# Unalome81/IEEE-802.11-OFDM-QPSK-Simulator

Measured on NVIDIA B200. Metric: OFDM symbols/s, TX+AWGN+RX chain (BER/EVM sweep), higher is better.
Workload: dtype f32+f64

## Files before the change

ieee-802.11-ofdm-qpsk-simulator_b200/binding.py:

```python
import ctypes as C
import os

import numpy as np

HERE = os.path.dirname(os.path.abspath(__file__))
LIB_PATH = os.path.join(HERE, "libofdm_b200.so")

MODE_EXACT, MODE_FAST = 0, 1
NFFT, CP, SYM_LEN, LTS_LEN, DATA_PER_SYM, BITS_PER_SYM, WORDS_PER_SYM = 64, 16, 80, 160, 48, 96, 3


def frame_len(n_sym):
    return LTS_LEN + SYM_LEN * n_sym


class Counters(C.Structure):
    _fields_ = [("bit_errors", C.c_uint64), ("bits", C.c_uint64), ("frames_in_error", C.c_uint64),
                ("rail_errors", C.c_uint64), ("frames", C.c_uint64),
                ("sum_err2", C.c_double), ("sum_ref2", C.c_double), ("sum_evm_lin", C.c_double)]

    def as_dict(self):
        return {k: getattr(self, k) for k, _ in self._fields_}

    def __iadd__(self, o):
# ... 31 lines not shown
    pass


_VP, _I, _L, _F, _U32, _U64, _SZ = C.c_void_p, C.c_int, C.c_long, C.c_float, C.c_uint32, C.c_uint64, C.c_size_t

SIGNATURES = {
    "ofdm_version": (_I, []),
    "ofdm_strerror": (C.c_char_p, [_I]),
    "ofdm_ctx_create": (_I, [C.POINTER(_VP), _I]),
    "ofdm_ctx_destroy": (_I, [_VP]),
    "ofdm_last_error": (C.c_char_p, [_VP]),
    "ofdm_ctx_set_stream": (_I, [_VP, _VP]),
    "ofdm_ctx_stream": (_VP, [_VP]),
    "ofdm_ctx_sync": (_I, [_VP]),
    "ofdm_ctx_set_option": (_I, [_VP, C.c_char_p, _I]),
    "ofdm_ctx_replayed_frames": (_I, [_VP, C.POINTER(_U64), _I]),
    "ofdm_ctx_sm_count": (_I, [_VP]),
    "ofdm_ctx_launch_count": (_U64, [_VP]),
    "ofdm_dev_alloc": (_I, [_VP, C.POINTER(_VP), _SZ]),
    "ofdm_dev_free": (_I, [_VP, _VP]),
    "ofdm_host_alloc": (_I, [_VP, C.POINTER(_VP), _SZ]),
    "ofdm_host_free": (_I, [_VP, _VP]),
    "ofdm_memcpy_h2d": (_I, [_VP, _VP, _VP, _SZ]),
    "ofdm_memcpy_d2h": (_I, [_VP, _VP, _VP, _SZ]),
    "ofdm_memset_dev": (_I, [_VP, _VP, _I, _SZ]),
    "ofdm_pack_bits": (_I, [_VP, _VP, _VP, _L]),
    "ofdm_unpack_bits": (_I, [_VP, _VP, _VP, _L]),
    "ofdm_qpsk_modulate": (_I, [_VP, _VP, _VP, _L]),
    "ofdm_map_subcarriers": (_I, [_VP, _VP, _VP, _L]),
    "ofdm_ifft64": (_I, [_VP, _VP, _VP, _L, _I]),
    "ofdm_fft64": (_I, [_VP, _VP, _VP, _L, _I]),
    "ofdm_add_cp": (_I, [_VP, _VP, _VP, _L]),
    "ofdm_lts": (_I, [_VP, _VP, _VP]),
    "ofdm_tx_frames": (_I, [_VP, _VP, _VP, _VP, _L, _I, _I]),
    "ofdm_frame_power": (_I, [_VP, _VP, _VP, _L, _I, _I]),
    "ofdm_awgn_inject": (_I, [_VP, _VP, _VP, _VP, _F, _VP, _L, _I, _I]),
    "ofdm_awgn_philox": (_I, [_VP, _VP, _VP, _F, _U32, _U32, _U64, _VP, _L, _I, _I]),
    "ofdm_awgn_philox_ex": (_I, [_VP, _I, _I, _VP, _VP, _F, _U32, _U32, _U64, _VP, _L, _I, _I]),
    "ofdm_rx_frames": (_I, [_VP, _VP, _VP, _L, _I, _I, _VP, C.POINTER(RxDump)]),
    "ofdm_awgn_rx_inject": (_I, [_VP, _VP, _VP, _VP, _VP, _F, _L, _I, _I, _VP, C.POINTER(RxDump)]),
    "ofdm_awgn_rx_philox": (_I, [_VP, _VP, _VP, _VP, _F, _U32, _U32, _U64, _L, _I, _I, _VP, C.POINTER(RxDump)]),
    "ofdm_awgn_rx_inject_sweep": (_I, [_VP, _VP, _VP, _VP, _VP, _VP, _I, _L, _I, _I, _VP]),
    "ofdm_strip_cp": (_I, [_VP, _VP, _VP, _L, _I, _I, _I]),
    "ofdm_channel_estimate": (_I, [_VP, _VP, _VP, _L, _I, _I, _I]),
    "ofdm_equalize": (_I, [_VP, _VP, _VP, _VP, _L, _I, _I]),
    "ofdm_demap": (_I, [_VP, _VP, _VP, _L]),
    "ofdm_agc_slicer": (_I, [_VP, _VP, _VP, _L]),
    "ofdm_qpsk_demodulate": (_I, [_VP, _VP, _VP, _L]),
    "ofdm_sweep_inject_host": (_I, [_VP, _VP, _VP, _L, _I, _VP, _I, _I, C.POINTER(Counters)]),
    "ofdm_sweep_inject_dev": (_I, [_VP, _VP, _VP, _L, _I, _VP, _I, _I, C.POINTER(Counters)]),
    "ofdm_random_bits": (_I, [_VP, _U32, _U64, _L, _I, _VP]),
    "ofdm_mc_sweep_philox_dev": (_I, [_VP, _U32, _U64, _L, _I, _VP, _I, _I, _VP]),
    "ofdm_mc_sweep_points_dev": (_I, [_VP, _U32, _U64, _L, _I, _I, _VP, _VP, _I, _I, _VP]),
    "ofdm_mc_sweep_until": (_I, [_VP, _U32, _U64, _I, _I, _VP, _I, _I, _U64, _U64, _L, C.POINTER(Counters), C.POINTER(_I)]),
    "ofdm_mc_sweep_channel_dev": (_I, [_VP, C.POINTER(Channel), _U32, _U64, _L, _I, _VP, _VP, _I, _I, _VP]),
    "ofdm_mc_sweep_channel_until": (_I, [_VP, C.POINTER(Channel), _U32, _U64, _I, _VP, _I, _I, _U64, _U64, _L, C.POINTER(Counters),
                                         C.POINTER(_I)]),
    "ofdm_mc_sweep_philox": (_I, [_VP, _U32, _U64, _L, _I, _VP, _I, _I, C.POINTER(Counters)]),
    "ofdm_multipath_taps": (_I, [_VP, _VP, _VP, _I, _VP, _L, _I]),
    "ofdm_multipath_philox": (_I, [_VP, _VP, _U32, _U64, _I, _VP, _VP, _L, _I]),
    "ofdm_mc_sweep_multipath_dev": (_I, [_VP, _U32, _U64, _L, _I, _I, _VP, _I, _I, _VP]),
    "ofdm_rrc_tx": (_I, [_VP, _VP, _VP, _L, _I]),
    "ofdm_rrc_rx": (_I, [_VP, _VP, _VP, _L, _I, _I, _I]),
    "ofdm_awgn_inject_len": (_I, [_VP, _VP, _VP, _VP, _F, _VP, _L, _I, _I]),
    "ofdm_packet_detect": (_I, [_VP, _VP, _VP, _L, _I]),
    "ofdm_packet_select": (_I, [_VP, _VP, _VP, _L, _I]),
# ... 447 lines not shown
```

ieee-802.11-ofdm-qpsk-simulator_b200/csrc/ofdm_b200.cu:

```cuda
#include <cmath>
#include <cstdio>
#include <cstdlib>
#include <cstring>
#include <mutex>
#include <new>
#include <set>
#include <type_traits>
#include <utility>

#include "ofdm_chain.cuh"
#include "ofdm_stream.cuh"
#include "ofdm_mc_quad.cuh"
#include "ofdm_sweep.cuh"

using namespace ofdm;

struct ofdm_ctx {
    int device = 0;
    int sm_count = 0;
    cudaStream_t stream = nullptr;
    bool owns_stream = false;
    cudaStream_t copy_stream = nullptr;
    cudaEvent_t copy_done[2] = {nullptr, nullptr}, call_start = nullptr;
    uint64_t launches = 0;
// ... 85 lines not shown
int stream_grid(ofdm_ctx *ctx, long rows, int rows_per_block, int per_sm)
{
    const long need = (rows + rows_per_block - 1) / rows_per_block, full = (long)per_sm * ctx->sm_count;
    const long g = need < full ? need : full;
    return (int)(g < 1 ? 1 : g);
}

int ensure_scratch(ofdm_ctx *ctx, int slot, size_t bytes, void **out)
{
    if (ctx->scratch_bytes[slot] < bytes) {
        if (ctx->scratch[slot]) { cudaFree(ctx->scratch[slot]); ctx->scratch[slot] = nullptr; ctx->scratch_bytes[slot] = 0; }
        cudaError_t e = cudaMalloc(&ctx->scratch[slot], bytes);
        if (e != cudaSuccess) return fail(ctx, OFDM_ERR_NOMEM, "cudaMalloc(scratch)", e);
        ctx->scratch_bytes[slot] = bytes;
    }
    *out = ctx->scratch[slot];
    return OFDM_OK;
}

float snr_linear(float snr_db)
{
    return (float)pow(10.0, (double)(snr_db / 10));
}

__global__ void k_power_prefix(const float2 *__restrict__ x, int n, float *__restrict__ out)
{
    float p = 0.f;
    for (int i = 0; i < n; ++i) {
        const double h = hypot_glibc((double)x[i].x, (double)x[i].y);
        p = __double2float_rn(__dadd_rn((double)p, __dmul_rn(h, h)));
    }
    *out = p;
}

struct DeviceTables {
    bool ready = false;
    float lts_freq[128], lts_time[320], sts_time[320], lts_power_prefix;
};
std::mutex g_tables_mutex;
DeviceTables g_tables[64];

int upload_tables(ofdm_ctx *ctx, const float *lts_time , float power_prefix)
{
    Tables t;
    memset(&t, 0, sizeof t);
    for (int k = 0; k < 32; ++k) t.tw64[k] = make_double2(kTw64[k][0], kTw64[k][1]);
    for (int k = 0; k < 64; ++k) {
        double a = 2.0 * 3.14159265358979323846 * k / 64.0;
        t.tw64f[k] = make_float2((float)cos(a), (float)(-sin(a)));
    }
    signed char by_c[64];
    for (int c = 0; c < 64; ++c) by_c[c] = -1;
    const int lo[6] = {6, 12, 26, 33, 40, 54}, hi[6] = {10, 24, 31, 38, 52, 58};
    int d = 0;
    for (int r = 0; r < 6; ++r) for (int c = lo[r]; c <= hi[r]; ++c) by_c[c] = (signed char)d++;
    by_c[11] = -2; by_c[25] = -2; by_c[39] = -2; by_c[53] = -3;
    for (int p = 0; p < 64; ++p) {
        int c = (p + 32) & 63;
        t.bin_data[p] = by_c[c];
        t.bin_lts[p] = (c >= 6 && c <= 58) ? kLk[c - 6] : 0;
        if (by_c[c] >= 0) t.data_bin[by_c[c]] = (int8_t)p;
    }
    if (lts_time) {
        memcpy(t.lts_time, lts_time, sizeof t.lts_time);
        double sum = 0.0;
        for (int i = 0; i < 160; ++i) sum += (double)lts_time[2 * i] * lts_time[2 * i] + (double)lts_time[2 * i + 1] * lts_time[2 * i + 1];
// ... 185 lines not shown
    std::lock_guard<std::mutex> lock(g_tables_mutex);
    DeviceTables &dt = g_tables[device & 63];
    int st = OFDM_OK;
    float *d_buf = nullptr;
    if (dt.ready) {
        memcpy(ctx->lts_freq, dt.lts_freq, sizeof dt.lts_freq);
        memcpy(ctx->lts_time, dt.lts_time, sizeof dt.lts_time);
        memcpy(ctx->sts_time, dt.sts_time, sizeof dt.sts_time);
        ctx->lts_power_prefix = dt.lts_power_prefix;
    } else {
    st = upload_tables(ctx, nullptr, 0.f);
    if (st == OFDM_OK && cudaMalloc(&d_buf, (2 * 128 + 320 + 4) * sizeof(float)) != cudaSuccess) st = OFDM_ERR_NOMEM;
    if (st == OFDM_OK) {
        memset(ctx->lts_freq, 0, sizeof ctx->lts_freq);
        for (int i = 0; i < 53; ++i) ctx->lts_freq[2 * (6 + i)] = (float)kLk[i];
        float t64[128];
        if (cudaMemcpyAsync(d_buf, ctx->lts_freq, sizeof ctx->lts_freq, cudaMemcpyHostToDevice, ctx->stream) != cudaSuccess) st = OFDM_ERR_CUDA;
        if (st == OFDM_OK) st = launch_fft<true, true>(ctx, d_buf, d_buf + 128, 1);
        if (st == OFDM_OK && cudaMemcpyAsync(t64, d_buf + 128, sizeof t64, cudaMemcpyDeviceToHost, ctx->stream) != cudaSuccess) st = OFDM_ERR_CUDA;
        if (st == OFDM_OK && cudaStreamSynchronize(ctx->stream) != cudaSuccess) st = OFDM_ERR_CUDA;
        if (st == OFDM_OK) {
            memcpy(ctx->lts_time, t64 + 64, 32 * 2 * sizeof(float));
            memcpy(ctx->lts_time + 64, t64, 64 * 2 * sizeof(float));
            memcpy(ctx->lts_time + 64 + 128, t64, 64 * 2 * sizeof(float));
            float *d_lts = d_buf + 256, *d_pref = d_buf + 256 + 320;
            if (cudaMemcpyAsync(d_lts, ctx->lts_time, sizeof ctx->lts_time, cudaMemcpyHostToDevice, ctx->stream) != cudaSuccess) st = OFDM_ERR_CUDA;
            if (st == OFDM_OK) {
                k_power_prefix<<<1, 1, 0, ctx->stream>>>(reinterpret_cast<const float2 *>(d_lts), 160, d_pref);
                st = check_launch(ctx, "k_power_prefix");
            }
            if (st == OFDM_OK && cudaMemcpyAsync(&ctx->lts_power_prefix, d_pref, sizeof(float), cudaMemcpyDeviceToHost, ctx->stream) != cudaSuccess) st = OFDM_ERR_CUDA;
            if (st == OFDM_OK && cudaStreamSynchronize(ctx->stream) != cudaSuccess) st = OFDM_ERR_CUDA;
            if (st == OFDM_OK) st = upload_tables(ctx, ctx->lts_time, ctx->lts_power_prefix);
        }
    }
    if (st == OFDM_OK) {
        static const signed char Sk[53] = {0,0,1,0,0,0,-1,0,0,0, 1,0,0,0,-1,0,0,0,-1,0,0,0, 1,0,0,0,0,0,0,0,-1,0,0,0, -1,0,0,0,1,0,0,0,1,0,0,0, 1,0,0,0,1,0,0};
        const float scale = (float)sqrt(13.0 / 6.0);
        float grid[128], t64[128];
        memset(grid, 0, sizeof grid);
        for (int i = 0; i < 53; ++i) { grid[2 * (6 + i)] = (float)Sk[i] * scale; grid[2 * (6 + i) + 1] = (float)Sk[i] * scale; }
        if (cudaMemcpyAsync(d_buf, grid, sizeof grid, cudaMemcpyHostToDevice, ctx->stream) != cudaSuccess) st = OFDM_ERR_CUDA;
        if (st == OFDM_OK) st = launch_fft<true, true>(ctx, d_buf, d_buf + 128, 1);
        if (st == OFDM_OK && cudaMemcpyAsync(t64, d_buf + 128, sizeof t64, cudaMemcpyDeviceToHost, ctx->stream) != cudaSuccess) st = OFDM_ERR_CUDA;
        if (st == OFDM_OK && cudaStreamSynchronize(ctx->stream) != cudaSuccess) st = OFDM_ERR_CUDA;
        if (st == OFDM_OK) for (int r = 0; r < 10; ++r) memcpy(ctx->sts_time + 32 * r, t64, 16 * 2 * sizeof(float));
    }
    if (st == OFDM_OK) {
        memcpy(dt.lts_freq, ctx->lts_freq, sizeof dt.lts_freq);
        memcpy(dt.lts_time, ctx->lts_time, sizeof dt.lts_time);
        memcpy(dt.sts_time, ctx->sts_time, sizeof dt.sts_time);
        dt.lts_power_prefix = ctx->lts_power_prefix;
        dt.ready = true;
    }
    }
    if (st == OFDM_OK) {
        if (cudaMalloc(&ctx->replayed_dev, sizeof(unsigned long long)) != cudaSuccess) st = OFDM_ERR_NOMEM;
        else if (cudaMemset(ctx->replayed_dev, 0, sizeof(unsigned long long)) != cudaSuccess) st = OFDM_ERR_CUDA;
    }
    if (st == OFDM_OK) {
        if (cudaMalloc(&ctx->sts_dev, sizeof ctx->sts_time) != cudaSuccess) st = OFDM_ERR_NOMEM;
        else if (cudaMemcpy(ctx->sts_dev, ctx->sts_time, sizeof ctx->sts_time, cudaMemcpyHostToDevice) != cudaSuccess) st = OFDM_ERR_CUDA;
    }
    if (d_buf) cudaFree(d_buf);
    if (st != OFDM_OK) { ofdm_ctx_destroy(ctx); return st; }
    *out = ctx;
// ... 160 lines not shown
    return check_launch(ctx, "k_map_subcarriers");
}
int ofdm_ifft64(ofdm_ctx *ctx, const float *in, float *out, long n, int mode)
{
    if (int st = bind(ctx)) return st;
    OFDM_REQUIRE(ctx, n >= 0 && mode_ok(mode));
    if (n == 0) return OFDM_OK;
    OFDM_REQUIRE(ctx, in != nullptr && out != nullptr && in != out);
    return mode == OFDM_MODE_EXACT ? launch_fft<true, true>(ctx, in, out, n) : launch_fft<false, true>(ctx, in, out, n);
}
int ofdm_fft64(ofdm_ctx *ctx, const float *in, float *out, long n, int mode)
{
    if (int st = bind(ctx)) return st;
    OFDM_REQUIRE(ctx, n >= 0 && mode_ok(mode));
    if (n == 0) return OFDM_OK;
    OFDM_REQUIRE(ctx, in != nullptr && out != nullptr && in != out);
    return mode == OFDM_MODE_EXACT ? launch_fft<true, false>(ctx, in, out, n) : launch_fft<false, false>(ctx, in, out, n);
}
int ofdm_add_cp(ofdm_ctx *ctx, const float *sym, float *out, long n)
{
    if (int st = bind(ctx)) return st;
    OFDM_REQUIRE(ctx, n >= 0);
    if (n == 0) return OFDM_OK;
    OFDM_REQUIRE(ctx, sym != nullptr && out != nullptr);
    k_add_cp<<<stream_grid(ctx, n, kRows4, 4), kRows4 * 80, 0, ctx->stream>>>(reinterpret_cast<const float2 *>(sym), reinterpret_cast<float2 *>(out), n);
    return check_launch(ctx, "k_add_cp");
}
int ofdm_lts(ofdm_ctx *ctx, float *lts_freq_host, float *lts_time_host)
{
    if (!ctx) return OFDM_ERR_INVALID;
    if (lts_freq_host) memcpy(lts_freq_host, ctx->lts_freq, sizeof ctx->lts_freq);
    if (lts_time_host) memcpy(lts_time_host, ctx->lts_time, sizeof ctx->lts_time);
    return OFDM_OK;
}

int ofdm_frame_power(ofdm_ctx *ctx, const float *frames, float *power, long n_frames, int frame_len, int mode)
{
    if (int st = bind(ctx)) return st;
    OFDM_REQUIRE(ctx, n_frames >= 0 && frame_len >= 1 && frame_len <= OFDM_FRAME_LEN(OFDM_MAX_SYM) && mode_ok(mode));
    if (n_frames == 0) return OFDM_OK;
    OFDM_REQUIRE(ctx, frames != nullptr && power != nullptr);
    return frame_power(ctx, frames, power, n_frames, frame_len, mode);
}

int ofdm_tx_frames(ofdm_ctx *ctx, const uint32_t *bits, float *frames, float *power, long n_frames, int n_sym, int mode)
{
    if (int st = bind(ctx)) return st;
    OFDM_REQUIRE(ctx, n_frames >= 0 && nsym_ok(n_sym) && mode_ok(mode));
    if (n_frames == 0) return OFDM_OK;
    OFDM_REQUIRE(ctx, bits != nullptr && frames != nullptr);
    int st;
    if (n_sym == 2 && (uintptr_t)frames % 16 == 0 && !ctx->force_generic) {
        const size_t smem = tx2_smem_bytes();
        auto launch = [&](auto k) -> int {
            OFDM_CUDA(ctx, allow_smem(ctx, k, smem));
            int grid = grid_for(ctx, k, smem, kWarpsPerBlock * 2, n_frames);
            k<<<grid, kThreads, smem, ctx->stream>>>(bits, reinterpret_cast<float2 *>(frames), n_frames);
            return check_launch(ctx, "k_tx_frames2");
        };
        st = mode == OFDM_MODE_EXACT ? launch(k_tx_frames2<true>) : launch(k_tx_frames2<false>);
    } else if (mode == OFDM_MODE_EXACT) {
        int grid = grid_for(ctx, k_tx_frames<true>, 0, kWarpsPerBlock * 4, n_frames * n_sym);
        k_tx_frames<true><<<grid, kThreads, 0, ctx->stream>>>(bits, reinterpret_cast<float2 *>(frames), n_frames, n_sym);
        st = check_launch(ctx, "k_tx_frames<exact>");
    } else {
        int grid = grid_for(ctx, k_tx_frames<false>, 0, kWarpsPerBlock * 4, n_frames * n_sym);
// ... 781 lines not shown
```

ieee-802.11-ofdm-qpsk-simulator_b200/csrc/ofdm_device.cuh:

```cuda
#pragma once
#include <cuda_runtime.h>
#include <stdint.h>
#include "twiddles64.h"

namespace ofdm {

constexpr int kGroupPitch = 72;
constexpr int kWarpTile = 4 * kGroupPitch;
constexpr float kQpsk = 0.70710678118654752440f;

constexpr double kTw64[32][2] = { OFDM_TWIDDLE64_TABLE };
constexpr double kW8r = kTw64[8][0],   kW8i = kTw64[8][1];
constexpr double kW16r = kTw64[16][0], kW16i = kTw64[16][1];
constexpr double kW24r = kTw64[24][0], kW24i = kTw64[24][1];
constexpr double kW8rS = kTw64[8][0] * 0x1p896, kW8iS = kTw64[8][1] * 0x1p896;
constexpr double kW24rS = kTw64[24][0] * 0x1p896, kW24iS = kTw64[24][1] * 0x1p896;

struct Tables {
    double2 tw64[32];
    float2 tw64f[64];
    int8_t bin_data[64];
    int8_t bin_lts[64];
    int8_t data_bin[48];
    float2 lts_time[160];
    float lts_power_prefix;
    float lts_power_sum;
};
__constant__ Tables c_tab;

__device__ __forceinline__ int rev3(int v) { return ((v & 1) << 2) | (v & 2) | ((v >> 2) & 1); }

__device__ __forceinline__ float2 cadd(float2 a, float2 b) { return __fadd2_rn(a, b); }
__device__ __forceinline__ float2 csub(float2 a, float2 b) { return __fadd2_rn(a, make_float2(-b.x, -b.y)); }
__device__ __forceinline__ float2 cadd_mi(float2 a, float2 b) { return __fadd2_rn(a, make_float2(b.y, -b.x)); }
__device__ __forceinline__ float2 csub_mi(float2 a, float2 b) { return __fadd2_rn(a, make_float2(-b.y, b.x)); }
__device__ __forceinline__ float2 cmul(float2 a, float2 b)
{
    const float2 t = __fmul2_rn(make_float2(a.y, a.y), make_float2(b.y, b.x));
    return __ffma2_rn(make_float2(a.x, a.x), b, make_float2(-t.x, t.y));
}

__device__ __forceinline__ void bf_exact(float2 &e, float2 &o, double wr, double wi)
{
    double c = (double)o.x, d = (double)o.y;
    const float2 w = make_float2(__double2float_rn(__dsub_rn(__dmul_rn(wr, c), __dmul_rn(wi, d))),
                                 __double2float_rn(__dadd_rn(__dmul_rn(wr, d), __dmul_rn(wi, c))));
    const float2 a = e;
    e = cadd(a, w); o = csub(a, w);
}
constexpr double kTwScale = 0x1p896;
__device__ __forceinline__ double f2d_scaled(float x)
{
    const uint32_t u = __float_as_uint(x);
    const uint32_t hi = ((u << 1) >> 4) | (u & 0x80000000u);
    return __hiloint2double((int)hi, (int)(u << 29));
}
__device__ __forceinline__ void bf_exact_s(float2 &e, float2 &o, double wr, double wi)
{
    const double c = f2d_scaled(o.x), d = f2d_scaled(o.y);
// ... 204 lines not shown
```

ieee-802.11-ofdm-qpsk-simulator_b200/csrc/ofdm_sweep.cuh:

```cuda
#pragma once
#include "ofdm_chain.cuh"

namespace ofdm {

struct SweepParams {
    const float2 *in;
    const float *g;
    const float *power;
    const uint32_t *tx_bits;
    long n_frames;
    int n_snr;
    float radius_scale;
    float evm_guard;
    float snr_lin[kMaxSnr];
    ofdm_counters *counters;
    unsigned long long *replayed;
};

struct alignas(16) SweepWarp {
    float2 tile[kWarpTile];
    float2 fx[4][kWin];
    float2 fn[4][kWin];
    StreamStage<true> st[kStages];
    uint64_t bar[kStages];
// ... 6 lines not shown
    float r;
    asm("sqrt.approx.ftz.f32 %0, %1;" : "=f"(r) : "f"(fmaf(z.x, z.x, z.y * z.y)));
    return fmaf(r, 1.000004f, 2e-19f);
}

__constant__ unsigned char c_sweep_pair[32] = { 1,  2,  5,  8, 11, 16, 19, 41, 44, 45, 46, 52, 54, 55, 58, 63,
                                                3,  4, 10, 12, 17, 18, 22, 23, 25, 47, 48, 53, 56, 59, 61, 62};
__constant__ unsigned char c_sweep_single[16] = { 6, 14, 15, 20, 26, 40, 49, 50,    9, 13, 24, 38, 39, 42, 51, 60};

struct SweepItems {
    int bin[2];
    int f_off[3];
    float k4[3];
    int word[3];
    int shift[3];
};

__device__ __forceinline__ SweepItems make_sweep_items(int lane)
{
    SweepItems c;
    c.bin[0] = c_sweep_pair[lane];
    c.bin[1] = c_sweep_single[(lane >> 4) * 8 + (lane & 7)];
#pragma unroll
    for (int t = 0; t < 3; ++t) {
        const int bin = c.bin[t >> 1], sym = t == 2 ? (lane >> 3) & 1 : t;
        const int d = c_tab.bin_data[bin];
        c.f_off[t] = sym * kWin + bin;
        c.k4[t] = 4.f * (0.5f * (float)c_tab.bin_lts[bin]);
        c.word[t] = sym * 3 + (d >> 4);
        c.shift[t] = 2 * (d & 15);
    }
    return c;
}

constexpr int kSweepWarps = 6;

template <int ARITH>
__global__ void __launch_bounds__(kSweepWarps * 32, 2) k_sweep_lin(SweepParams p)
{
    constexpr int LEVEL = ARITH == kArithChecked ? 2 : 1;
    constexpr int kWarps = kSweepWarps;
    extern __shared__ __align__(128) unsigned char s_raw[];
    const int lane = threadIdx.x & 31, warp = threadIdx.x >> 5, grp = lane >> 3, u = lane & 7;
    const int warp_u = __shfl_sync(0xffffffffu, warp, 0);
    SweepWarp &ws = reinterpret_cast<SweepWarp *>(s_raw)[warp];
    SweepWarp &ws_u = reinterpret_cast<SweepWarp *>(s_raw)[warp_u];
    float2 *tile = ws.tile + grp * kGroupPitch;
    Tw<false> tw; tw.load(u);
    const SweepItems ic = make_sweep_items(lane);
    constexpr int len = 320;
    const long stride = (long)gridDim.x * kWarps;
    const long f_first = (long)blockIdx.x * kWarps + warp_u;
    const double q = (double)kQpsk;
    const double ref2_frame = 96.0 * (2.0 * q * q);
    const float inv_ref2 = (float)(1.0 / ref2_frame);
    constexpr uint32_t kBytes = 4 * 512 + 4 * 256;
    constexpr int kStep = 3;

    const uint32_t stage0 = tma::saddr(&ws_u.st[0]);
    const uint32_t bar0 = tma::saddr(&ws_u.bar[0]);
    auto issue = [&](long f, int s) {
        if (tma::elect_one()) {
            const uint32_t bar = bar0 + 8u * (uint32_t)s;
            const uint32_t dst = stage0 + (uint32_t)s * (uint32_t)sizeof(StreamStage<true>);
            const char *x = reinterpret_cast<const char *>(p.in) + f * (len * 8);
            const char *g = reinterpret_cast<const char *>(p.g) + f * (len * 4);
            const uint32_t gd = dst + 4 * kWin * 8;
            tma::expect_tx_addr(bar, kBytes);
            tma::bulk_addr(dst + 0 * kWin * 8, x + 32 * 8, 512, bar);
            tma::bulk_addr(dst + 1 * kWin * 8, x + 96 * 8, 512, bar);
            tma::bulk_addr(dst + 2 * kWin * 8, x + 176 * 8, 512, bar);
            tma::bulk_addr(dst + 3 * kWin * 8, x + 256 * 8, 512, bar);
            tma::bulk_addr(gd + 0 * kWin * 4, g + 32 * 4, 256, bar);
            tma::bulk_addr(gd + 1 * kWin * 4, g + 96 * 4, 256, bar);
            tma::bulk_addr(gd + 2 * kWin * 4, g + 176 * 4, 256, bar);
            tma::bulk_addr(gd + 3 * kWin * 4, g + 256 * 4, 256, bar);
        }
    };
    if (lane == 0) {
        for (int s = 0; s < kStages; ++s) tma::mbar_init(&ws.bar[s], 1);
        tma::fence_mbar_init();
    }
    __syncwarp();
    for (int s = 0; s < kStages; ++s)
        if (f_first + s * stride < p.n_frames) issue(f_first + s * stride, s);

    uint32_t m_i[2] = {0, 0}, m_q[2] = {0, 0}, m_b[2] = {0, 0}, m_ferr[2] = {0, 0};
    float m_e2[2] = {0.f, 0.f}, m_evm[2] = {0.f, 0.f};
    double d_e2[2] = {0.0, 0.0}, d_evm[2] = {0.0, 0.0};
    uint32_t n_done = 0;
    uint32_t k = 0;
    for (long f = f_first; f < p.n_frames; f += stride, ++k) {
        const int s = (int)(k & 1u);
        const uint32_t phase = (k >> 1) & 1u;
        const float P = p.power[f];
        const uint32_t *wb = p.tx_bits + f * 6;
        uint32_t txw[3];
#pragma unroll
        for (int t = 0; t < 3; ++t) txw[t] = wb[ic.word[t]];

        tma::wait_addr(bar0 + 8u * (uint32_t)s, phase);
        float2 v[8];
        float gz[8];
        float2 n2x = make_float2(0.f, 0.f);
        float n2g = 0.f;
#pragma unroll
        for (int i = 0; i < 8; ++i) {
            v[i] = ws.st[s].x[grp][u + 8 * i];
            gz[i] = ws.st[s].g[grp][u + 8 * i];
            n2x = __ffma2_rn(v[i], v[i], n2x);
            n2g = fmaf(gz[i], gz[i], n2g);
        }
        __syncwarp();
        if (f + kStages * stride < p.n_frames) issue(f + kStages * stride, s);
        fft64<false>(v, tw, tile, u);
#pragma unroll
        for (int j = 0; j < 8; ++j) ws.fx[grp][u + 8 * j] = v[j];
#pragma unroll
        for (int i = 0; i < 8; ++i) v[i] = make_float2(gz[i], 0.f);
        fft64<false>(v, tw, tile, u);
#pragma unroll
        for (int j = 0; j < 8; ++j) ws.fn[grp][u + 8 * j] = v[j];
        float2 nn = make_float2(n2x.x + n2x.y, n2g);
#pragma unroll
        for (int o = 1; o < 8; o <<= 1)
            nn = __fadd2_rn(nn, make_float2(__shfl_xor_sync(0xffffffffu, nn.x, o), __shfl_xor_sync(0xffffffffu, nn.y, o)));
        {
            float rx, rn;
            asm("sqrt.approx.ftz.f32 %0, %1;" : "=f"(rx) : "f"(nn.x));
            asm("sqrt.approx.ftz.f32 %0, %1;" : "=f"(rn) : "f"(nn.y));
            const bool ok = nn.x >= 1e-30f && nn.x < 1e20f && nn.y < 1e20f;
            const float inf = __int_as_float(0x7f800000);
            if (u == 0) { ws.norm[grp] = ok ? p.radius_scale * rx : inf; ws.norm[4 + grp] = ok ? p.radius_scale * rn : inf; }
        }
        __syncwarp();
        const float4 rX = *reinterpret_cast<const float4 *>(ws.norm), rN = *reinterpret_cast<const float4 *>(ws.norm + 4);
        const float rHX = rX.x + rX.y, rHN = rN.x + rN.y;
        float2 FX[3], FN[3], GX[2], GN[2];
        float c0[3], c1[3], c2[3], hcX[2], hcN[2];
#pragma unroll
        for (int e = 0; e < 2; ++e) {
            const int bin = ic.bin[e];
            GX[e] = cadd(ws.fx[0][bin], ws.fx[1][bin]);
            GN[e] = cadd(ws.fn[0][bin], ws.fn[1][bin]);
            if (LEVEL >= 2) { hcX[e] = modulus_up(GX[e]); hcN[e] = modulus_up(GN[e]); }
        }
#pragma unroll
        for (int t = 0; t < 3; ++t) {
            FX[t] = (&ws.fx[2][0])[ic.f_off[t]];
            FN[t] = (&ws.fn[2][0])[ic.f_off[t]];
            const bool sym0 = ic.f_off[t] < kWin;
            const float rFX = sym0 ? rX.z : rX.w, rFN = sym0 ? rN.z : rN.w;
            if (LEVEL >= 2) {
                const float faX = modulus_up(FX[t]), faN = modulus_up(FN[t]);
                const float hX = hcX[t >> 1], hN = hcN[t >> 1];
                const float A0 = hX + rHX, A1 = hN + rHN;
                c0[t] = fmaf(rFX, A0, fmaf(rHX, faX, 1.2e-7f * (faX * hX)));
                c1[t] = fmaf(rFX, A1, fmaf(rFN, A0, fmaf(rHX, faN, fmaf(rHN, faX, 1.2e-7f * fmaf(faX, hN, faN * hX)))));
                c2[t] = fmaf(rFN, A1, fmaf(rHN, faN, 1.2e-7f * (faN * hN)));
            } else { c0[t] = c1[t] = c2[t] = 0.f; }
        }
        __syncwarp();
        uint32_t gq[3];
#pragma unroll
        for (int t = 0; t < 3; ++t) {
            const uint32_t tp = txw[t] >> ic.shift[t];
            const uint32_t kb = __float_as_uint(ic.k4[t]) & 0x80000000u;
            const uint32_t fq = (tp << 31) ^ kb, fi = ((tp ^ (tp >> 1)) << 31) ^ kb;
            gq[t] = (tp >> 1) << 31;
            FX[t] = make_float2(__uint_as_float(__float_as_uint(FX[t].x) ^ fi), __uint_as_float(__float_as_uint(FX[t].y) ^ fq));
            FN[t] = make_float2(__uint_as_float(__float_as_uint(FN[t].x) ^ fi), __uint_as_float(__float_as_uint(FN[t].y) ^ fq));
        }
#pragma unroll
        for (int e = 0; e < 2; ++e) {
            GX[e].y = __uint_as_float(__float_as_uint(GX[e].y) ^ gq[2 * e]);
            GN[e].y = __uint_as_float(__float_as_uint(GN[e].y) ^ gq[2 * e]);
        }
        const uint32_t g_rel = gq[0] ^ gq[1];
        float sig_lo = 0.f, sig_hi = 0.f;
        if (lane < p.n_snr) sig_lo = __fsqrt_rn(__fdiv_rn(P, p.snr_lin[lane]));
        if (p.n_snr > 32 && lane + 32 < p.n_snr) sig_hi = __fsqrt_rn(__fdiv_rn(P, p.snr_lin[lane + 32]));
        auto sig_pos = [](int i) { return (i / 3) * 4 + i % 3; };
        float *sigs = reinterpret_cast<float *>(&ws.fn[1][0]);
// ... 168 lines not shown
```

include/ofdm_b200.h:

```cpp
#ifndef OFDM_B200_H
#define OFDM_B200_H

#include <stddef.h>
#include <stdint.h>

#ifdef __cplusplus
extern "C" {
#endif

#define OFDM_B200_VERSION 100

enum {
    OFDM_OK = 0,
    OFDM_ERR_INVALID = 1,
    OFDM_ERR_CUDA = 2,
    OFDM_ERR_NOMEM = 3,
    OFDM_ERR_IO = 4,
    OFDM_ERR_NODEVICE = 5
};

enum { OFDM_MODE_EXACT = 0, OFDM_MODE_FAST = 1 };

#define OFDM_NFFT 64
#define OFDM_CP 16
// ... 25 lines not shown
    uint32_t *bits;
    int32_t *frame_bit_errors;
    float *frame_evm_lin;
} ofdm_rx_dump;

int ofdm_version(void);
const char *ofdm_strerror(int status);
int ofdm_ctx_create(ofdm_ctx **ctx, int device);
int ofdm_ctx_destroy(ofdm_ctx *ctx);
const char *ofdm_last_error(const ofdm_ctx *ctx);
int ofdm_ctx_set_stream(ofdm_ctx *ctx, void *cuda_stream);
void *ofdm_ctx_stream(const ofdm_ctx *ctx);
int ofdm_ctx_sync(ofdm_ctx *ctx);
int ofdm_ctx_set_option(ofdm_ctx *ctx, const char *name, int value);
int ofdm_ctx_replayed_frames(ofdm_ctx *ctx, uint64_t *count, int reset);
int ofdm_ctx_sm_count(const ofdm_ctx *ctx);
uint64_t ofdm_ctx_launch_count(const ofdm_ctx *ctx);
int ofdm_dev_alloc(ofdm_ctx *ctx, void **ptr, size_t bytes);
int ofdm_dev_free(ofdm_ctx *ctx, void *ptr);
int ofdm_host_alloc(ofdm_ctx *ctx, void **ptr, size_t bytes);
int ofdm_host_free(ofdm_ctx *ctx, void *ptr);
int ofdm_memcpy_h2d(ofdm_ctx *ctx, void *dst_dev, const void *src_host, size_t bytes);
int ofdm_memcpy_d2h(ofdm_ctx *ctx, void *dst_host, const void *src_dev, size_t bytes);
int ofdm_memset_dev(ofdm_ctx *ctx, void *dst_dev, int value, size_t bytes);

int ofdm_pack_bits(ofdm_ctx *ctx, const uint8_t *bits_dev, uint32_t *packed_dev, long n_symbols);
int ofdm_unpack_bits(ofdm_ctx *ctx, const uint32_t *packed_dev, uint8_t *bits_dev, long n_symbols);
int ofdm_qpsk_modulate(ofdm_ctx *ctx, const uint32_t *bits_dev, float *mod_dev, long n_symbols);
int ofdm_map_subcarriers(ofdm_ctx *ctx, const float *mod_dev, float *grid_dev, long n_symbols);
int ofdm_ifft64(ofdm_ctx *ctx, const float *in_dev, float *out_dev, long n, int mode);
int ofdm_fft64(ofdm_ctx *ctx, const float *in_dev, float *out_dev, long n, int mode);
int ofdm_add_cp(ofdm_ctx *ctx, const float *sym_dev, float *out_dev, long n);
int ofdm_lts(ofdm_ctx *ctx, float *lts_freq_host, float *lts_time_host);
int ofdm_tx_frames(ofdm_ctx *ctx, const uint32_t *bits_dev, float *frames_dev, float *power_dev,
                   long n_frames, int n_sym, int mode);
int ofdm_frame_power(ofdm_ctx *ctx, const float *frames_dev, float *power_dev, long n_frames, int frame_len, int mode);
int ofdm_awgn_inject(ofdm_ctx *ctx, const float *tx_dev, const float *g_dev, const float *power_dev, float snr_db,
                     float *ota_dev, long n_frames, int n_sym, int mode);
int ofdm_awgn_philox(ofdm_ctx *ctx, const float *tx_dev, const float *power_dev, float snr_db, uint32_t seed,
                     uint32_t stream, uint64_t frame0, float *ota_dev, long n_frames, int n_sym, int mode);

enum { OFDM_NOISE_REAL_RAIL = 0, OFDM_NOISE_COMPLEX = 1 };
enum { OFDM_SNR_FRAME_POWER = 0, OFDM_SNR_ESN0 = 1, OFDM_SNR_EBN0 = 2 };
typedef struct { int noise, snr_def, n_taps; } ofdm_channel;
int ofdm_awgn_philox_ex(ofdm_ctx *ctx, int noise, int snr_def, const float *tx_dev, const float *power_dev, float snr_db,
                        uint32_t seed, uint32_t stream, uint64_t frame0, float *ota_dev, long n_frames, int n_sym, int mode);
int ofdm_rx_frames(ofdm_ctx *ctx, const float *ota_dev, const uint32_t *tx_bits_dev, long n_frames, int n_sym,
                   int mode, ofdm_counters *counters_dev, const ofdm_rx_dump *dump);
int ofdm_awgn_rx_inject(ofdm_ctx *ctx, const float *tx_dev, const float *g_dev, const float *power_dev,
                        const uint32_t *tx_bits_dev, float snr_db, long n_frames, int n_sym, int mode,
                        ofdm_counters *counters_dev, const ofdm_rx_dump *dump);
int ofdm_awgn_rx_philox(ofdm_ctx *ctx, const float *tx_dev, const float *power_dev, const uint32_t *tx_bits_dev,
                        float snr_db, uint32_t seed, uint32_t stream, uint64_t frame0, long n_frames, int n_sym,
                        int mode, ofdm_counters *counters_dev, const ofdm_rx_dump *dump);

int ofdm_awgn_rx_inject_sweep(ofdm_ctx *ctx, const float *tx_dev, const float *g_dev, const float *power_dev,
                              const uint32_t *tx_bits_dev, const float *snr_db, int n_snr, long n_frames, int n_sym, int mode,
                              ofdm_counters *counters_dev);

int ofdm_strip_cp(ofdm_ctx *ctx, const float *frames_dev, float *bodies_dev, long n_frames, int n_sym, int frame_len, int data_off);
int ofdm_channel_estimate(ofdm_ctx *ctx, const float *frames_dev, float *H_dev, long n_frames, int frame_len, int lts_off, int mode);
int ofdm_equalize(ofdm_ctx *ctx, const float *F_dev, const float *H_dev, float *E_dev, long n_frames, int n_sym, int mode);
int ofdm_demap(ofdm_ctx *ctx, const float *grid_dev, float *points_dev, long n_symbols);
int ofdm_agc_slicer(ofdm_ctx *ctx, const float *points_dev, float *sliced_dev, long n_symbols);
int ofdm_qpsk_demodulate(ofdm_ctx *ctx, const float *points_dev, uint32_t *bits_dev, long n_symbols);

// ... 61 lines not shown
```

Before: 10.58 billion.

## Reuse precomputed LTS spectrum and pack real noise FFTs in sweep kernel

At init, the FFT of the standard LTS, its moduli and norms are computed once and stored in constant memory. The sweep kernel compares each frame's LTS samples bit-for-bit against the standard pattern. When they match, it reuses the cached spectrum instead of transforming the LTS. It then packs the two real noise rails into single complex FFTs and separates them with conjugate symmetry, cutting per-frame FFT work. The cost is a per-frame compare, extra shared-memory tables, a second code path and changed norm-bound arithmetic for the split transforms, which could alter rounding or bounds.

```diff
diff --git a/ieee-802.11-ofdm-qpsk-simulator_b200/binding.py b/ieee-802.11-ofdm-qpsk-simulator_b200/binding.py
--- a/ieee-802.11-ofdm-qpsk-simulator_b200/binding.py
+++ b/ieee-802.11-ofdm-qpsk-simulator_b200/binding.py
@@ -87,6 +87,7 @@
     "ofdm_fft64": (_I, [_VP, _VP, _VP, _L, _I]),
     "ofdm_add_cp": (_I, [_VP, _VP, _VP, _L]),
     "ofdm_lts": (_I, [_VP, _VP, _VP]),
+    "ofdm_sweep_lts_terms": (_I, [_VP, _VP, _VP]),
     "ofdm_tx_frames": (_I, [_VP, _VP, _VP, _VP, _L, _I, _I]),
     "ofdm_frame_power": (_I, [_VP, _VP, _VP, _L, _I, _I]),
     "ofdm_awgn_inject": (_I, [_VP, _VP, _VP, _VP, _F, _VP, _L, _I, _I]),
diff --git a/ieee-802.11-ofdm-qpsk-simulator_b200/csrc/ofdm_b200.cu b/ieee-802.11-ofdm-qpsk-simulator_b200/csrc/ofdm_b200.cu
--- a/ieee-802.11-ofdm-qpsk-simulator_b200/csrc/ofdm_b200.cu
+++ b/ieee-802.11-ofdm-qpsk-simulator_b200/csrc/ofdm_b200.cu
@@ -141,6 +141,10 @@
     }
     *out = p;
 }
+
+constexpr size_t kLtsTermsBytes = 194 * sizeof(float);
+static_assert(offsetof(Tables, lts_gx_mod) == offsetof(Tables, lts_gx) + 128 * sizeof(float) &&
+              offsetof(Tables, lts_norm) == offsetof(Tables, lts_gx) + 192 * sizeof(float), "LTS terms layout");
 
 struct DeviceTables {
     bool ready = false;
@@ -392,6 +396,13 @@
             if (st == OFDM_OK && cudaMemcpyAsync(&ctx->lts_power_prefix, d_pref, sizeof(float), cudaMemcpyDeviceToHost, ctx->stream) != cudaSuccess) st = OFDM_ERR_CUDA;
             if (st == OFDM_OK && cudaStreamSynchronize(ctx->stream) != cudaSuccess) st = OFDM_ERR_CUDA;
             if (st == OFDM_OK) st = upload_tables(ctx, ctx->lts_time, ctx->lts_power_prefix);
+            if (st == OFDM_OK) {
+                k_sweep_lts_terms<<<1, 32, 0, ctx->stream>>>(reinterpret_cast<const float2 *>(d_lts) + 32, d_buf);
+                st = check_launch(ctx, "k_sweep_lts_terms");
+            }
+            if (st == OFDM_OK && cudaMemcpyToSymbolAsync(c_tab, d_buf, kLtsTermsBytes, offsetof(Tables, lts_gx), cudaMemcpyDeviceToDevice,
+                                                         ctx->stream) != cudaSuccess) st = OFDM_ERR_CUDA;
+            if (st == OFDM_OK && cudaStreamSynchronize(ctx->stream) != cudaSuccess) st = OFDM_ERR_CUDA;
         }
     }
     if (st == OFDM_OK) {
@@ -618,6 +629,25 @@
     if (lts_freq_host) memcpy(lts_freq_host, ctx->lts_freq, sizeof ctx->lts_freq);
     if (lts_time_host) memcpy(lts_time_host, ctx->lts_time, sizeof ctx->lts_time);
     return OFDM_OK;
+}
+
+int ofdm_sweep_lts_terms(ofdm_ctx *ctx, const float *frame, float *out)
+{
+    if (int st = bind(ctx)) return st;
+    OFDM_REQUIRE(ctx, out != nullptr);
+    if (!frame) {
+        OFDM_CUDA(ctx, cudaMemcpyFromSymbolAsync(out, c_tab, kLtsTermsBytes, offsetof(Tables, lts_gx), cudaMemcpyDeviceToHost, ctx->stream));
+        OFDM_CUDA(ctx, cudaStreamSynchronize(ctx->stream));
+        return OFDM_OK;
+    }
+    float *d_out = nullptr;
+    OFDM_CUDA(ctx, cudaMalloc(&d_out, kLtsTermsBytes));
+    k_sweep_lts_terms<<<1, 32, 0, ctx->stream>>>(reinterpret_cast<const float2 *>(frame) + 32, d_out);
+    int st = check_launch(ctx, "k_sweep_lts_terms");
+    if (st == OFDM_OK && cudaMemcpyAsync(out, d_out, kLtsTermsBytes, cudaMemcpyDeviceToHost, ctx->stream) != cudaSuccess) st = OFDM_ERR_CUDA;
+    if (st == OFDM_OK && cudaStreamSynchronize(ctx->stream) != cudaSuccess) st = OFDM_ERR_CUDA;
+    cudaFree(d_out);
+    return st == OFDM_ERR_CUDA ? fail(ctx, st, "ofdm_sweep_lts_terms") : st;
 }
 
 int ofdm_frame_power(ofdm_ctx *ctx, const float *frames, float *power, long n_frames, int frame_len, int mode)
diff --git a/ieee-802.11-ofdm-qpsk-simulator_b200/csrc/ofdm_device.cuh b/ieee-802.11-ofdm-qpsk-simulator_b200/csrc/ofdm_device.cuh
--- a/ieee-802.11-ofdm-qpsk-simulator_b200/csrc/ofdm_device.cuh
+++ b/ieee-802.11-ofdm-qpsk-simulator_b200/csrc/ofdm_device.cuh
@@ -25,6 +25,9 @@
     float2 lts_time[160];
     float lts_power_prefix;
     float lts_power_sum;
+    float2 lts_gx[64];
+    float lts_gx_mod[64];
+    float lts_norm[2];
 };
 __constant__ Tables c_tab;
 
diff --git a/ieee-802.11-ofdm-qpsk-simulator_b200/csrc/ofdm_sweep.cuh b/ieee-802.11-ofdm-qpsk-simulator_b200/csrc/ofdm_sweep.cuh
--- a/ieee-802.11-ofdm-qpsk-simulator_b200/csrc/ofdm_sweep.cuh
+++ b/ieee-802.11-ofdm-qpsk-simulator_b200/csrc/ofdm_sweep.cuh
@@ -62,6 +62,44 @@
     }
     return c;
 }
+
+__global__ void __launch_bounds__(32) k_sweep_lts_terms(const float2 *lts , float *out)
+{
+    __shared__ float2 tile[kWarpTile];
+    __shared__ float2 fx[2][kWin];
+    const int lane = threadIdx.x & 31, grp = lane >> 3, u = lane & 7;
+    Tw<false> tw; tw.load(u);
+    float2 v[8];
+    float2 n2x = make_float2(0.f, 0.f);
+#pragma unroll
+    for (int i = 0; i < 8; ++i) {
+        v[i] = grp < 2 ? lts[grp * 64 + u + 8 * i] : make_float2(0.f, 0.f);
+        n2x = __ffma2_rn(v[i], v[i], n2x);
+    }
+    fft64<false>(v, tw, tile + grp * kGroupPitch, u);
+    if (grp < 2) {
+#pragma unroll
+        for (int j = 0; j < 8; ++j) fx[grp][u + 8 * j] = v[j];
+    }
+    float2 nn = make_float2(n2x.x + n2x.y, 0.f);
+#pragma unroll
+    for (int o = 1; o < 8; o <<= 1)
+        nn = __fadd2_rn(nn, make_float2(__shfl_xor_sync(0xffffffffu, nn.x, o), __shfl_xor_sync(0xffffffffu, nn.y, o)));
+    float rx;
+    asm("sqrt.approx.ftz.f32 %0, %1;" : "=f"(rx) : "f"(nn.x));
+    const bool ok = nn.x >= 1e-30f && nn.x < 1e20f;
+    if (u == 0 && grp < 2) out[192 + grp] = ok ? rx : __int_as_float(0x7f800000);
+    __syncwarp();
+#pragma unroll
+    for (int h = 0; h < 2; ++h) {
+        const int bin = lane + 32 * h;
+        const float2 G = cadd(fx[0][bin], fx[1][bin]);
+        out[2 * bin] = G.x; out[2 * bin + 1] = G.y;
+        out[128 + bin] = modulus_up(G);
+    }
+}
+
+constexpr float kSplitRadZ = 124.f / 320.f, kSplitRadS = 176.f / 320.f;
 
 constexpr int kSweepWarps = 6;
 
@@ -111,7 +149,18 @@
         for (int s = 0; s < kStages; ++s) tma::mbar_init(&ws.bar[s], 1);
         tma::fence_mbar_init();
     }
-    __syncwarp();
+    __shared__ float4 s_lts[64];
+    __shared__ float2 s_gx[64];
+    __shared__ float s_gxm[64];
+    if (LEVEL >= 2) {
+        for (int i = threadIdx.x; i < 64; i += blockDim.x) {
+            const float2 a = c_tab.lts_time[32 + 2 * i], b = c_tab.lts_time[33 + 2 * i];
+            s_lts[i] = make_float4(a.x, a.y, b.x, b.y);
+            s_gx[i] = c_tab.lts_gx[i];
+            s_gxm[i] = c_tab.lts_gx_mod[i];
+        }
+        __syncthreads();
+    }
     for (int s = 0; s < kStages; ++s)
         if (f_first + s * stride < p.n_frames) issue(f_first + s * stride, s);
 
@@ -130,55 +179,133 @@
         for (int t = 0; t < 3; ++t) txw[t] = wb[ic.word[t]];
 
         tma::wait_addr(bar0 + 8u * (uint32_t)s, phase);
-        float2 v[8];
-        float gz[8];
-        float2 n2x = make_float2(0.f, 0.f);
-        float n2g = 0.f;
-#pragma unroll
-        for (int i = 0; i < 8; ++i) {
-            v[i] = ws.st[s].x[grp][u + 8 * i];
-            gz[i] = ws.st[s].g[grp][u + 8 * i];
-            n2x = __ffma2_rn(v[i], v[i], n2x);
-            n2g = fmaf(gz[i], gz[i], n2g);
-        }
-        __syncwarp();
-        if (f + kStages * stride < p.n_frames) issue(f + kStages * stride, s);
-        fft64<false>(v, tw, tile, u);
-#pragma unroll
-        for (int j = 0; j < 8; ++j) ws.fx[grp][u + 8 * j] = v[j];
-#pragma unroll
-        for (int i = 0; i < 8; ++i) v[i] = make_float2(gz[i], 0.f);
-        fft64<false>(v, tw, tile, u);
-#pragma unroll
-        for (int j = 0; j < 8; ++j) ws.fn[grp][u + 8 * j] = v[j];
-        float2 nn = make_float2(n2x.x + n2x.y, n2g);
-#pragma unroll
-        for (int o = 1; o < 8; o <<= 1)
-            nn = __fadd2_rn(nn, make_float2(__shfl_xor_sync(0xffffffffu, nn.x, o), __shfl_xor_sync(0xffffffffu, nn.y, o)));
-        {
-            float rx, rn;
-            asm("sqrt.approx.ftz.f32 %0, %1;" : "=f"(rx) : "f"(nn.x));
-            asm("sqrt.approx.ftz.f32 %0, %1;" : "=f"(rn) : "f"(nn.y));
-            const bool ok = nn.x >= 1e-30f && nn.x < 1e20f && nn.y < 1e20f;
-            const float inf = __int_as_float(0x7f800000);
-            if (u == 0) { ws.norm[grp] = ok ? p.radius_scale * rx : inf; ws.norm[4 + grp] = ok ? p.radius_scale * rn : inf; }
-        }
-        __syncwarp();
+        bool std_lts = false;
+        if (LEVEL >= 2) {
+            const float4 *w = reinterpret_cast<const float4 *>(&ws.st[s].x[lane >> 4][4 * (lane & 15)]);
+            const float4 a = w[0], b = w[1], ea = s_lts[2 * lane], eb = s_lts[2 * lane + 1];
+            uint32_t d = (__float_as_uint(a.x) ^ __float_as_uint(ea.x)) | (__float_as_uint(a.y) ^ __float_as_uint(ea.y));
+            d |= (__float_as_uint(a.z) ^ __float_as_uint(ea.z)) | (__float_as_uint(a.w) ^ __float_as_uint(ea.w));
+            d |= (__float_as_uint(b.x) ^ __float_as_uint(eb.x)) | (__float_as_uint(b.y) ^ __float_as_uint(eb.y));
+            d |= (__float_as_uint(b.z) ^ __float_as_uint(eb.z)) | (__float_as_uint(b.w) ^ __float_as_uint(eb.w));
+            std_lts = __all_sync(0xffffffffu, d == 0u);
+        }
+        const float inf = __int_as_float(0x7f800000);
+        float2 FX[3], FN[3], GX[2], GN[2];
+        float hcX[2];
+        if (std_lts) {
+            float2 v[8];
+            float2 n2 = make_float2(0.f, 0.f);
+            if (grp < 2) {
+#pragma unroll
+                for (int i = 0; i < 8; ++i) { v[i] = ws.st[s].x[2 + grp][u + 8 * i]; n2 = __ffma2_rn(v[i], v[i], n2); }
+            } else {
+                const float *ga = ws.st[s].g[grp == 2 ? 2 : 0], *gb = ws.st[s].g[grp == 2 ? 3 : 1];
+                const float2 sel = grp == 2 ? make_float2(0.f, 1.f) : make_float2(1.f, 0.f);
+#pragma unroll
+                for (int i = 0; i < 8; ++i) {
+                    const float2 ab = make_float2(ga[u + 8 * i], gb[u + 8 * i]);
+                    v[i] = __ffma2_rn(make_float2(ab.y, ab.y), sel, make_float2(ab.x, 0.f));
+                    n2 = __ffma2_rn(ab, ab, n2);
+                }
+            }
+            __syncwarp();
+            if (f + kStages * stride < p.n_frames) issue(f + kStages * stride, s);
+            fft64<false>(v, tw, tile, u);
+#pragma unroll
+            for (int j = 0; j < 8; ++j) ws.fx[grp][u + 8 * j] = v[j];
+            float2 nn = grp < 2 ? make_float2(n2.x + n2.y, 0.f) : n2;
+#pragma unroll
+            for (int o = 1; o < 8; o <<= 1)
+                nn = __fadd2_rn(nn, make_float2(__shfl_xor_sync(0xffffffffu, nn.x, o), __shfl_xor_sync(0xffffffffu, nn.y, o)));
+            {
+                float r0, r1, rz;
+                asm("sqrt.approx.ftz.f32 %0, %1;" : "=f"(r0) : "f"(nn.x));
+                asm("sqrt.approx.ftz.f32 %0, %1;" : "=f"(r1) : "f"(nn.y));
+                asm("sqrt.approx.ftz.f32 %0, %1;" : "=f"(rz) : "f"(nn.x + nn.y));
+                const bool clean = grp < 2, split = grp == 2;
+                const bool ok = clean ? nn.x >= 1e-30f && nn.x < 1e20f : nn.x < 1e20f && nn.y < 1e20f;
+                const float cz = split ? kSplitRadZ : 0.f, cs = split ? kSplitRadS : 1.f;
+                const float va = fmaf(cz, rz, cs * r0);
+                const float vb = clean ? c_tab.lts_norm[grp & 1] : fmaf(cz, rz, cs * r1);
+                const int sa = clean ? 2 + grp : split ? 6 : 4, sb = clean ? grp : sa + 1;
+                if (u == 0) {
+                    ws.norm[sa] = ok ? p.radius_scale * va : inf;
+                    ws.norm[sb] = ok || clean ? p.radius_scale * vb : inf;
+                }
+            }
+            __syncwarp();
+#pragma unroll
+            for (int e = 0; e < 2; ++e) {
+                const int bin = ic.bin[e];
+                GX[e] = s_gx[bin];
+                GN[e] = ws.fx[3][bin];
+                if (LEVEL >= 2) hcX[e] = s_gxm[bin];
+            }
+#pragma unroll
+            for (int t = 0; t < 3; ++t) {
+                const int bin = ic.bin[t >> 1];
+                FX[t] = (&ws.fx[0][0])[ic.f_off[t]];
+                const float2 zk = ws.fx[2][bin], zm = ws.fx[2][(64 - bin) & 63];
+                const bool sym1 = t == 2 ? ((lane >> 3) & 1) != 0 : t == 1;
+                const float2 a = sym1 ? make_float2(zk.y, -zk.x) : zk, b = sym1 ? make_float2(zm.y, zm.x) : make_float2(zm.x, -zm.y);
+                FN[t] = __fmul2_rn(__fadd2_rn(a, b), make_float2(0.5f, 0.5f));
+            }
+        } else {
+            float2 v[8];
+            float gz[8];
+            float2 n2x = make_float2(0.f, 0.f);
+            float n2g = 0.f;
+#pragma unroll
+            for (int i = 0; i < 8; ++i) {
+                v[i] = ws.st[s].x[grp][u + 8 * i];
+                gz[i] = ws.st[s].g[grp][u + 8 * i];
+                n2x = __ffma2_rn(v[i], v[i], n2x);
+                n2g = fmaf(gz[i], gz[i], n2g);
+            }
+            __syncwarp();
+            if (f + kStages * stride < p.n_frames) issue(f + kStages * stride, s);
+            fft64<false>(v, tw, tile, u);
+#pragma unroll
+            for (int j = 0; j < 8; ++j) ws.fx[grp][u + 8 * j] = v[j];
+#pragma unroll
+            for (int i = 0; i < 8; ++i) v[i] = make_float2(gz[i], 0.f);
+            fft64<false>(v, tw, tile, u);
+#pragma unroll
+            for (int j = 0; j < 8; ++j) ws.fn[grp][u + 8 * j] = v[j];
+            float2 nn = make_float2(n2x.x + n2x.y, n2g);
+#pragma unroll
+            for (int o = 1; o < 8; o <<= 1)
+                nn = __fadd2_rn(nn, make_float2(__shfl_xor_sync(0xffffffffu, nn.x, o), __shfl_xor_sync(0xffffffffu, nn.y, o)));
+            {
+                float rx, rn;
+                asm("sqrt.approx.ftz.f32 %0, %1;" : "=f"(rx) : "f"(nn.x));
+                asm("sqrt.approx.ftz.f32 %0, %1;" : "=f"(rn) : "f"(nn.y));
+                const bool ok = nn.x >= 1e-30f && nn.x < 1e20f && nn.y < 1e20f;
+                if (u == 0) { ws.norm[grp] = ok ? p.radius_scale * rx : inf; ws.norm[4 + grp] = ok ? p.radius_scale * rn : inf; }
+            }
+            __syncwarp();
+#pragma unroll
+            for (int e = 0; e < 2; ++e) {
+                const int bin = ic.bin[e];
+                GX[e] = cadd(ws.fx[0][bin], ws.fx[1][bin]);
+                GN[e] = cadd(ws.fn[0][bin], ws.fn[1][bin]);
+                if (LEVEL >= 2) hcX[e] = modulus_up(GX[e]);
+            }
+#pragma unroll
+            for (int t = 0; t < 3; ++t) {
+                FX[t] = (&ws.fx[2][0])[ic.f_off[t]];
+                FN[t] = (&ws.fn[2][0])[ic.f_off[t]];
+            }
+        }
         const float4 rX = *reinterpret_cast<const float4 *>(ws.norm), rN = *reinterpret_cast<const float4 *>(ws.norm + 4);
         const float rHX = rX.x + rX.y, rHN = rN.x + rN.y;
-        float2 FX[3], FN[3], GX[2], GN[2];
-        float c0[3], c1[3], c2[3], hcX[2], hcN[2];
-#pragma unroll
-        for (int e = 0; e < 2; ++e) {
-            const int bin = ic.bin[e];
-            GX[e] = cadd(ws.fx[0][bin], ws.fx[1][bin]);
-            GN[e] = cadd(ws.fn[0][bin], ws.fn[1][bin]);
-            if (LEVEL >= 2) { hcX[e] = modulus_up(GX[e]); hcN[e] = modulus_up(GN[e]); }
+        float c0[3], c1[3], c2[3], hcN[2];
+        if (LEVEL >= 2) {
+#pragma unroll
+            for (int e = 0; e < 2; ++e) hcN[e] = modulus_up(GN[e]);
         }
 #pragma unroll
         for (int t = 0; t < 3; ++t) {
-            FX[t] = (&ws.fx[2][0])[ic.f_off[t]];
-            FN[t] = (&ws.fn[2][0])[ic.f_off[t]];
             const bool sym0 = ic.f_off[t] < kWin;
             const float rFX = sym0 ? rX.z : rX.w, rFN = sym0 ? rN.z : rN.w;
             if (LEVEL >= 2) {
diff --git a/include/ofdm_b200.h b/include/ofdm_b200.h
--- a/include/ofdm_b200.h
+++ b/include/ofdm_b200.h
@@ -81,6 +81,7 @@
 int ofdm_fft64(ofdm_ctx *ctx, const float *in_dev, float *out_dev, long n, int mode);
 int ofdm_add_cp(ofdm_ctx *ctx, const float *sym_dev, float *out_dev, long n);
 int ofdm_lts(ofdm_ctx *ctx, float *lts_freq_host, float *lts_time_host);
+int ofdm_sweep_lts_terms(ofdm_ctx *ctx, const float *frame_dev, float *out_host);
 int ofdm_tx_frames(ofdm_ctx *ctx, const uint32_t *bits_dev, float *frames_dev, float *power_dev,
                    long n_frames, int n_sym, int mode);
 int ofdm_frame_power(ofdm_ctx *ctx, const float *frames_dev, float *power_dev, long n_frames, int frame_len, int mode);
```

After: 10.50 billion (median of 6 runs). About the same (-0.8%).
